# GJ0407790/cuda_ray_tracer

Measured on AMD Instinct MI355X. Metric: Mrays/sec, tenthousand.txt 1080p@16spp, higher is better.
Workload: dtype f32

## Files before the change

### cuda_ray_tracer_amd/csrc/api.hip

```cpp
#include "scene_dev.h"
#include "host_scene.h"

#include <cmath>
#include <cstdlib>
#include <cstring>
#include <new>
#include <string>
#include <vector>

using namespace mirt;

namespace {

template <typename T>
int upload(T** dst, const std::vector<T>& src)
{
  *dst = nullptr;
  if (src.empty()) return MIRT_OK;
  MIRT_HIP(hipMalloc(dst, sizeof(T) * src.size()));
  MIRT_HIP(hipMemcpy(*dst, src.data(), sizeof(T) * src.size(), hipMemcpyHostToDevice));
  return MIRT_OK;
}

bool nonzero(const MirtRGB& c) { return !(fabsf(c.r) < 1e-6f && fabsf(c.g) < 1e-6f && fabsf(c.b) < 1e-6f); }
// ... 151 lines not shown
  if (!std::isfinite(d->expose) && d->expose != INFINITY) sc->colors_finite = false;
  std::vector<LightDev> suns((size_t)d->num_suns), bulbs((size_t)d->num_bulbs);
  for (int i = 0; i < d->num_suns; ++i) {
    const MirtVec3& v = d->suns[i].dir;
    const float mag = sqrtf(v.x * v.x + v.y * v.y + v.z * v.z);
    float nx = 0.0f, ny = 0.0f, nz = 0.0f;
    const float diff = fabsf(mag - 0.0f), largest = fmaxf(fabsf(mag), fabsf(0.0f));
    const bool zero = (largest < 1e-6f) ? (diff < 1e-6f) : (diff / largest < 1e-6f);
    if (!zero) { const float inv = 1.0f / mag; nx = v.x * inv; ny = v.y * inv; nz = v.z * inv; }
    suns[i] = {v.x, v.y, v.z, d->suns[i].color.r, d->suns[i].color.g, d->suns[i].color.b, nx, ny, nz, 1.0f / nx, 1.0f / ny, 1.0f / nz};
  }
  for (int i = 0; i < d->num_bulbs; ++i) bulbs[i] = {d->bulbs[i].point.x, d->bulbs[i].point.y, d->bulbs[i].point.z, d->bulbs[i].color.r, d->bulbs[i].color.g, d->bulbs[i].color.b, 0, 0, 0, 0, 0, 0};
  sc->d.spheres = nullptr; sc->d.triangles = nullptr; sc->d.prim_refs = nullptr; sc->d.planes = nullptr; sc->d.suns = nullptr; sc->d.bulbs = nullptr;

  int rc = MIRT_OK;
  auto chk = [&](int r) { if (rc == MIRT_OK) rc = r; };
  {
    const size_t nodes_bytes = N > 1 ? 64 * (size_t)(N - 1) : 0;
    const size_t sph_bytes = 16 * (size_t)sc->Ns, tri_bytes = 48 * (size_t)sc->Nt;
    const size_t qnode_bytes = (sc->Nt == 0 && N > 1) ? 32 * (size_t)(N - 1) : 0;
    const size_t wnode_bytes = (sc->Nt > 0 && N > 1) ? 64 * (size_t)(N - 1) + 128 : 0;
    const size_t total = nodes_bytes + sph_bytes + tri_bytes + 64 + qnode_bytes + wnode_bytes;
    if (total > 0xfffffff0ull) { delete sc; set_error("mirt_scene_create: scene too large for 32-bit record offsets"); return MIRT_ERR_ARG; }
    hipError_t e = hipMalloc(&sc->heap, total);
    if (e == hipSuccess) e = hipMemset(sc->heap, 0, total);
    if (e != hipSuccess) { delete sc; return hip_fail(e, "hipMalloc(heap)", __FILE__, __LINE__); }
    sc->prim_base = (uint32_t)nodes_bytes;
    sc->qnode_base = qnode_bytes ? (uint32_t)(nodes_bytes + sph_bytes + tri_bytes + 64) : 0u;
    sc->wnode_base = wnode_bytes ? (uint32_t)((nodes_bytes + sph_bytes + tri_bytes + 64 + qnode_bytes + 127) / 128 * 128) : 0u;
    sc->nodes = reinterpret_cast<float4*>(sc->heap);
  }
  chk(upload(&sc->spheres, spheres)); chk(upload(&sc->tris, tris));
  chk(upload(&sc->tri_verts, verts)); chk(upload(&sc->mats, mats));
  chk(upload(&sc->refs_in, refs)); chk(upload(&sc->planes, planes)); chk(upload(&sc->suns, suns)); chk(upload(&sc->bulbs, bulbs));
  auto alloc = [&](void** p, size_t bytes) { if (rc == MIRT_OK && bytes) { hipError_t e = hipMalloc(p, bytes); if (e != hipSuccess) rc = hip_fail(e, "hipMalloc", __FILE__, __LINE__); } };
  if (N > 0) {
    alloc((void**)&sc->codes, 4 * (size_t)N); alloc((void**)&sc->order, 4 * (size_t)N);
    alloc((void**)&sc->parent, 4 * (2 * (size_t)N - 1)); alloc((void**)&sc->boxes, 24 * (2 * (size_t)N - 1));
    if (N > 1) { alloc((void**)&sc->child_l, 4 * (size_t)(N - 1)); alloc((void**)&sc->child_r, 4 * (size_t)(N - 1)); alloc((void**)&sc->range, 8 * (size_t)(N - 1)); }
    alloc((void**)&sc->unit_prim, 4 * ((size_t)sc->Ns + 3 * (size_t)sc->Nt));
    alloc((void**)&sc->tris_before, 4 * ((size_t)N + 1));
  }
  alloc((void**)&sc->bounds_keys, 6 * 4);
  alloc((void**)&sc->qparams, 9 * 4);
  alloc((void**)&sc->tri_boxes, 32 * (size_t)sc->Nt);
  for (int i = 0; i < mirt::MIRT_MAX_FRAMES; ++i) {
    alloc((void**)&sc->ctx[i].counters, 16 * sizeof(unsigned long long));
    if (rc == MIRT_OK && hipMemset(sc->ctx[i].counters, 0, 16 * sizeof(unsigned long long)) != hipSuccess) rc = MIRT_ERR_HIP;
  }
  if (rc == MIRT_OK) {
    hipError_t e = hipEventCreate(&sc->ev0);
    if (e == hipSuccess) e = hipEventCreate(&sc->ev1);
    if (e == hipSuccess) e = hipEventCreate(&sc->so_ev);
    for (int i = 0; i < mirt::MIRT_MAX_FRAMES && e == hipSuccess; ++i) {
      e = hipEventCreate(&sc->ctx[i].ev0);
      if (e == hipSuccess) e = hipEventCreate(&sc->ctx[i].ev1);
      if (e == hipSuccess) e = hipEventCreate(&sc->ctx[i].ev2);
      if (e == hipSuccess) e = hipEventCreate(&sc->ctx[i].ev3);
      if (e == hipSuccess) e = hipEventCreate(&sc->ctx[i].order_ev);
    }
    if (e != hipSuccess) rc = hip_fail(e, "hipEventCreate", __FILE__, __LINE__);
  }
  if (rc != MIRT_OK) { mirt_scene_destroy(sc); return rc; }
  *out = sc;
  return MIRT_OK;
}

}

extern "C" {

void mirt_scene_destroy(MirtScene* sc)
{
  if (!sc) return;
  hipSetDevice(sc->device);
  hipDeviceSynchronize();
  hipFree(sc->heap); hipFree(sc->spheres); hipFree(sc->tris); hipFree(sc->tri_verts); hipFree(sc->mats); hipFree(sc->refs_in);
  hipFree(sc->unit_prim); hipFree(sc->tris_before); hipFree(sc->range);
  hipFree(sc->planes); hipFree(sc->suns); hipFree(sc->bulbs);
  hipFree(sc->codes); hipFree(sc->order); hipFree(sc->child_l); hipFree(sc->child_r); hipFree(sc->parent); hipFree(sc->boxes); hipFree(sc->build_ws);
  hipFree(sc->bounds_keys); hipFree(sc->qparams); hipFree(sc->tri_boxes);
  for (int i = 0; i < mirt::MIRT_MAX_FRAMES; ++i) {
    mirt::RenderCtx& c = sc->ctx[i];
    hipFree(c.samples); hipFree(c.stack_spill); hipFree(c.pending); hipFree(c.counters); hipFree(c.args_dev);
    hipFree(c.chunk_cost); for (uint32_t* o : c.order_out) hipFree(o);
    hipFree(c.sp_list); hipFree(c.sp_table); hipFree(c.sp_blocks);
    if (c.ev0) hipEventDestroy(c.ev0);
    if (c.ev1) hipEventDestroy(c.ev1);
    if (c.ev2) hipEventDestroy(c.ev2);
    if (c.ev3) hipEventDestroy(c.ev3);
    if (c.order_ev) hipEventDestroy(c.order_ev);
    for (hipEvent_t e : c.slab_ev) hipEventDestroy(e);
  }
  rng_cache_free(&sc->rng);
  hipFree(sc->wf_state); hipFree(sc->wf_rays); hipFree(sc->wf_ctr);
  if (sc->wf_ctr_host) hipHostFree(sc->wf_ctr_host);
  for (hipEvent_t e : sc->wf_events) hipEventDestroy(e);
  if (sc->ev0) hipEventDestroy(sc->ev0);
  if (sc->ev1) hipEventDestroy(sc->ev1);
  if (sc->so_ev) hipEventDestroy(sc->so_ev);
  hipFree(sc->so_order); hipFree(sc->so_keys); hipFree(sc->so_keys2); hipFree(sc->so_ws);
  delete sc;
}

int mirt_build_lbvh(MirtScene* sc, void* stream, float* build_ms)
{
  if (!sc) { set_error("mirt_build_lbvh: null scene"); return MIRT_ERR_ARG; }
  MIRT_HIP(hipSetDevice(sc->device));
  int rc = build_lbvh(sc, (hipStream_t)stream);
  if (rc == MIRT_OK) sc->updated = false;
  if (rc == MIRT_OK && build_ms) *build_ms = sc->build_ms;
  return rc;
}

int64_t mirt_render_num_pixels(const MirtRenderParams* p) { return p ? render_num_pixels(p) : -1; }

int mirt_part_pixel_xy(const MirtRenderParams* p, int64_t local, int32_t* x, int32_t* y)
{
  if (!p) { set_error("mirt_part_pixel_xy: null argument"); return MIRT_ERR_ARG; }
  return part_pixel(p, local, x, y);
}

int mirt_render(MirtScene* sc, const MirtRenderParams* p, void* d_rgba8, void* d_rgba_f32, void* stream)
{
  if (!sc || !p) { set_error("mirt_render: null argument"); return MIRT_ERR_ARG; }
  MIRT_HIP(hipSetDevice(sc->device));
  return render(sc, p, d_rgba8, d_rgba_f32, (hipStream_t)stream);
}

int mirt_render_accumulate(MirtScene* sc, const MirtRenderParams* p, void* d_accum_f32, int sample_first, int sample_count, void* stream)
{
  if (!sc || !p) { set_error("mirt_render_accumulate: null argument"); return MIRT_ERR_ARG; }
  MIRT_HIP(hipSetDevice(sc->device));
  return render_accumulate(sc, p, d_accum_f32, sample_first, sample_count, (hipStream_t)stream);
}

int mirt_finalize(const MirtRenderParams* p, const void* d_accum_f32, int total_samples, void* d_rgba8, void* stream)
{
  if (!p) { set_error("mirt_finalize: null argument"); return MIRT_ERR_ARG; }
  return finalize(p, d_accum_f32, total_samples, d_rgba8, (hipStream_t)stream);
}

int mirt_render_accumulate_pixels(MirtScene* sc, const MirtRenderParams* p, const uint32_t* d_pixels, int64_t num_listed, void* d_accum_f32,
                                  void* d_accum_sq_f32, uint32_t* d_counts, int sample_first, int sample_count, void* stream)
{
  if (!sc || !p) { set_error("mirt_render_accumulate_pixels: null argument"); return MIRT_ERR_ARG; }
  if (!d_pixels && num_listed > 0) { set_error("mirt_render_accumulate_pixels: null pixel list (every pixel of the part: d_pixels = NULL with num_listed = 0)"); return MIRT_ERR_ARG; }
  MIRT_HIP(hipSetDevice(sc->device));
  mirt::AdaptiveArgs ax;
  ax.list = d_pixels; ax.num_listed = num_listed; ax.accum_sq = (float4*)d_accum_sq_f32; ax.counts = d_counts;
  return render_accumulate_pixels(sc, p, ax, d_accum_f32, sample_first, sample_count, (hipStream_t)stream);
}

int mirt_select_pixels(const MirtRenderParams* p, const void* d_accum_f32, const void* d_accum_sq_f32, const uint32_t* d_counts, int min_samples,
                       int max_samples, float max_variance, uint32_t* d_pixels_out, uint32_t* d_num_out, void* stream)
{
  if (!p) { set_error("mirt_select_pixels: null argument"); return MIRT_ERR_ARG; }
  return select_pixels(p, d_accum_f32, d_accum_sq_f32, d_counts, min_samples, max_samples, max_variance, d_pixels_out, d_num_out, (hipStream_t)stream);
}

int mirt_finalize_counts(const MirtRenderParams* p, const void* d_accum_f32, const uint32_t* d_counts, void* d_rgba8, void* stream)
{
  if (!p) { set_error("mirt_finalize_counts: null argument"); return MIRT_ERR_ARG; }
  return finalize_counts(p, d_accum_f32, d_counts, d_rgba8, (hipStream_t)stream);
}

int mirt_scatter_part(const MirtRenderParams* p, const void* d_part_rgba8, void* d_frame_rgba8, void* stream)
// ... 124 lines not shown
```

### cuda_ray_tracer_amd/csrc/render.hip

```cpp
#include "scene_dev.h"
#include "host_scene.h"
#include "shade_common.h"

#include <algorithm>
#include <climits>
#include <cmath>
#include <cstdio>
#include <cstdlib>
#include <cstring>

namespace mirt {
namespace {

constexpr int RBLOCK = 256;
constexpr int MAX_SPP = 4096;
constexpr int MAX_SLAB_ARGS = 4;
#ifndef MIRT_TRACE_BLOCK
#define MIRT_TRACE_BLOCK 64
#endif
constexpr int TRACE_BLOCK = MIRT_TRACE_BLOCK;
constexpr int MAX_CHUNK_SHIFT = 8, MIN_CHUNK_SHIFT = 6;
#ifndef MIRT_WAVES_PER_SIMD
#define MIRT_WAVES_PER_SIMD 4
#endif
#ifndef MIRT_STACK_LDS
#define MIRT_STACK_LDS 24
#endif
constexpr int STACK_LDS = MIRT_STACK_LDS;
MIRT_DEV bool triangle_leaf_reached(const RenderArgs* __restrict__ ap, uint32_t off16, const f3& o, const f3& d, float t, float tmin, f3& inv)
{
  const RenderArgs* aq = ap;
  asm volatile("" : "+s"(aq));
  const uint32_t id = aq->unit_prim[off16 - aq->prim_base16] & 0x7fffffffu;
  const float4 b0 = aq->tri_boxes[2 * (size_t)id], b1 = aq->tri_boxes[2 * (size_t)id + 1];
  inv = mk3(1.0f / d.x, 1.0f / d.y, 1.0f / d.z);
  const float tx1 = (b0.x - o.x) * inv.x, tx2 = (b0.y - o.x) * inv.x;
  const float ty1 = (b0.z - o.y) * inv.y, ty2 = (b0.w - o.y) * inv.y;
  const float tz1 = (b1.x - o.z) * inv.z, tz2 = (b1.y - o.z) * inv.z;
  const float te = fmaxf(fmaxf(fminf(tx1, tx2), fminf(ty1, ty2)), fminf(tz1, tz2));
  const float tx = fminf(fminf(fmaxf(tx1, tx2), fmaxf(ty1, ty2)), fmaxf(tz1, tz2));
  return te < tx && tx > tmin && te < t;
}

template <bool COUNT, int TABLES, bool QN, int SPECX = 0>
__global__ void __launch_bounds__(TRACE_BLOCK, MIRT_WAVES_PER_SIMD) trace_kernel(const RenderArgs* __restrict__ ap, const HotArgs h)
{
  constexpr int SPEC = SPECX;
  constexpr bool NOTRI = (SPEC & SPEC_NOTRI) != 0;
  constexpr bool WIDE = QN && !NOTRI;
#define MIRT_HELD (QN && !(SPEC & SPEC_NOBULB) && h.reach_check && S.batch_pending && !S.trav && S.li >= h.num_suns && S.li < h.num_suns + h.num_bulbs && \
                   S.refbest != REF_NONE)
  __shared__ __attribute__((aligned(16))) unsigned char lds_raw[STACK_LDS * TRACE_BLOCK * 4];
  __shared__ uint4 lds_rng[2][TRACE_BLOCK];
  __shared__ uint4 lds_park[2][TRACE_BLOCK];
  uint32_t* const lds_stack = reinterpret_cast<uint32_t*>(lds_raw);
  const int tid = threadIdx.x;
  const int lane = tid & 63;
  (void)lane;
  const unsigned char* const heap = reinterpret_cast<const unsigned char*>(h.nodes);
  const uint32_t gid32 = blockIdx.x * (uint32_t)TRACE_BLOCK + (uint32_t)tid;
  const long long gid = (long long)gid32;
  const long long gthreads = (long long)(gridDim.x * (uint32_t)TRACE_BLOCK);
  Counters cn = {0, 0, 0, 0, 0, 0, 0, 0, 0};

  unsigned long long c_next = 0, c_end = 0;
  bool exhausted = false;

  Lane S;
  S.g = -1; S.trav = false;
  S.rng.v0 = S.rng.v1 = S.rng.v2 = S.rng.v3 = S.rng.v4 = S.rng.d = 0; S.rng.bm_flag = 0; S.rng.bm_extra = 0.0f;
  S.L = mk3(0, 0, 0); S.alpha = 0.0f; S.steps = 0;
  S.Hdir = mk3(0, 0, 0); S.Hp = mk3(0, 0, 0); S.Hn = mk3(0, 0, 0); S.Hcolor = mk3(0, 0, 0);
  S.Hbounce = 0; S.Hior = 1.458f; S.Hrough = 0.0f; S.HtransNZ = false;
  S.wt = mk3(1, 1, 1); S.wD = mk3(0, 0, 0); S.pn = mk3(0, 0, 0);
  S.pc = 0; S.refr_bounce = 0; S.gi_n = 0; S.state = ST_PRIMARY;
  S.bo = mk3(0, 0, 0); S.rdir = mk3(0, 0, 1); S.li = 0; S.occl = 0ull; S.batch_pending = false; S.has_reflect = false;
  S.o = mk3(0, 0, 0); S.d = mk3(0, 0, 1); S.inv = mk3(0, 0, 1); S.bounce = 0; S.limit = INFINITY; S.shadow = false;
  S.tplane = INFINITY; S.plane_id = -1;
  S.qb = mk3(0, 0, 0); S.qc = mk3(0, 0, 0); S.qsx = S.qsy = S.qsz = 0;
  S.cur = REF_NONE; S.tos = REF_NONE; S.sp = 0; S.tbest = INFINITY; S.refbest = REF_NONE;

  lds_rng[0][tid] = make_uint4(0, 0, 0, 0);
  lds_rng[1][tid] = make_uint4(0, 0, 0, 0);
  lds_park[0][tid] = make_uint4(0, 0, 0, 0);
  lds_park[1][tid] = make_uint4(0, 0, 0, __float_as_uint(1.458f));
  for (;;) {
    const RenderArgs* aq = ap;
    asm volatile("" : "+s"(aq));
    const RenderArgs& a = *aq;
    if (a.reach_check && !S.trav && S.g >= 0 && !(exhausted && S.batch_pending && !MIRT_HELD) && (!S.batch_pending || S.li >= a.num_suns)) {
      if (hit_needs_literal_walk<QN>(a, S)) walk_literally<COUNT, NOTRI>(a, S, cn, gid, gthreads);
    }
    {
      const uint4 r0 = lds_rng[0][tid], r1 = lds_rng[1][tid];
      S.rng.v0 = r0.x; S.rng.v1 = r0.y; S.rng.v2 = r0.z; S.rng.v3 = r0.w;
      S.rng.v4 = r1.x; S.rng.d = r1.y; S.rng.bm_extra = __uint_as_float(r1.z); S.rng.bm_flag = (int)r1.w;
      const uint4 p0 = lds_park[0][tid], p1 = lds_park[1][tid];
      S.L = mk3(__uint_as_float(p0.x), __uint_as_float(p0.y), __uint_as_float(p0.z)); S.alpha = __uint_as_float(p0.w);
      S.wD = mk3(__uint_as_float(p1.x), __uint_as_float(p1.y), __uint_as_float(p1.z)); S.Hior = __uint_as_float(p1.w);
    }
    while (!S.trav && S.g >= 0 && !(exhausted && S.batch_pending && !MIRT_HELD)) {
      if (S.batch_pending) batch_next<COUNT, QN, RenderArgs, SPEC>(a, S, cn);
      else advance<COUNT, QN, SPEC>(a, S, cn, gid, gthreads);
    }
    if (!exhausted) {
      const unsigned long long need = __ballot(!S.trav && S.g < 0);
      if (need && (__popcll(need) >= a.init_k || __ballot(S.trav || S.batch_pending) == 0)) {
        const int want = __popcll(need);
        const unsigned long long nsamples = (unsigned long long)a.num_samples;
        const unsigned long long chunk = 1ull << a.chunk_shift;
        const unsigned long long nchunks = (nsamples + chunk - 1) >> a.chunk_shift;
        const int r = (int)__builtin_amdgcn_mbcnt_hi((unsigned)(need >> 32), __builtin_amdgcn_mbcnt_lo((unsigned)need, 0u));
        int given = 0;
        long long my = -1;
        while (given < want) {
          if (c_next >= c_end) {
            unsigned long long k = 0;
            if (lane == 0) {
              k = atomicAdd(a.work_counter, 1ull);
              if (k < nchunks && a.chunk_order) k = a.chunk_order[k];
            }
            k = __shfl(k, 0);
            if (k >= nchunks) {
              if (lane == 0 && atomicAdd(a.work_counter + 4, 1ull) == (unsigned long long)gridDim.x * (TRACE_BLOCK / 64) - 1ull) {
                a.work_counter[4] = 0ull;
                a.work_counter[0] = 0ull;
              }
              exhausted = true;
              break;
            }
            c_next = k << a.chunk_shift;
            c_end = (c_next + chunk < nsamples) ? c_next + chunk : nsamples;
          }
          const int avail = (int)(c_end - c_next);
          const int take = (want - given < avail) ? want - given : avail;
          if (!S.trav && S.g < 0 && r >= given && r < given + take) my = (long long)c_next + (r - given);
          c_next += (unsigned long long)take;
          given += take;
        }
        if (my >= 0) init_sample<COUNT, TABLES, QN>(a, S, cn, a.sample_order ? (long long)a.sample_order[my] : my);
      }
    }
    lds_rng[0][tid] = make_uint4(S.rng.v0, S.rng.v1, S.rng.v2, S.rng.v3);
    lds_rng[1][tid] = make_uint4(S.rng.v4, S.rng.d, __float_as_uint(S.rng.bm_extra), (uint32_t)S.rng.bm_flag);
    lds_park[0][tid] = make_uint4(__float_as_uint(S.L.x), __float_as_uint(S.L.y), __float_as_uint(S.L.z), __float_as_uint(S.alpha));
    lds_park[1][tid] = make_uint4(__float_as_uint(S.wD.x), __float_as_uint(S.wD.y), __float_as_uint(S.wD.z), __float_as_uint(S.Hior));
    if (__ballot(S.trav || S.batch_pending) == 0) {
      if (exhausted && __ballot(S.g >= 0) == 0) break;
      continue;
    }

    const float tmin = 0.0001f;
    for (;;) {
      const unsigned long long tm = __ballot(S.trav);
      const bool pend = !S.trav && S.batch_pending && !MIRT_HELD;
      const unsigned long long bm = __ballot(pend);
      if (tm == 0 && bm == 0) break;
      const int nwait = __popcll(__ballot(!S.trav && !pend && (S.g >= 0 || !exhausted)));
      const int nlive = __popcll(__ballot(S.g >= 0));
      const bool drain = exhausted && nlive <= h.drain_lanes;
      if (nwait >= h.refill_k || (drain && nwait > 0)) break;
      if (bm != 0 && (__popcll(bm) >= h.batch_k || tm == 0 || drain)) {
        if (pend) batch_next<COUNT, QN, HotArgs, SPEC>(h, S, cn);
      }
      const bool leaf0 = S.trav && (S.cur & REF_LEAF) != 0;
      const unsigned long long lm = __ballot(leaf0);
      const bool do_leaf0 = __popcll(lm) >= h.leaf_k || __ballot(S.trav && !leaf0) == 0 || drain;
      for (int rep = 0; rep < h.reps; ++rep) {
      const bool leaf = S.trav && (S.cur & REF_LEAF) != 0;
      const bool do_leaf = rep == 0 && do_leaf0;
      if (S.trav && (!leaf || do_leaf)) {
        if (COUNT) ++S.steps;
        const float4* rec = reinterpret_cast<const float4*>(heap + (S.cur << 4));
        bool pop = false;
        if (leaf) {
          float t = 0.0f;
          bool hit = false;
          const float4 q0 = rec[0];
          const bool tri = !NOTRI && (S.cur & REF_TRI) != 0;
          if (tri) {
            if (COUNT) cn.tri_tests++;
            const float4 q1 = rec[1], q2 = rec[2];
            hit = triangle_hit(q0, q1, q2, S.o, S.d, t);
          } else {
            if (COUNT) cn.sphere_tests++;
            float tc, t_far;
            hit = sphere_hit(q0, S.o, S.d, t, tc, t_far);
            if (QN && hit && (NOTRI || S.qsx != 0u)) hit = sphere_leaf_box_admits(q0, S.o, S.d, tc, t_far);
          }
          bool closer = closer_hit(hit, t, S.tbest, S.cur & REF_OFFMASK, S.refbest);
          if (QN && !NOTRI && closer && tri && S.qsx != 0u) {
            f3 inv;
            if (!triangle_leaf_reached(ap, S.cur & REF_OFFMASK, S.o, S.d, t, tmin, inv)) {
              closer = false;
              S.inv = inv; S.qsx = 0u;
              S.tos = 0u; S.sp = 1;
              S.tbest = INFINITY; S.refbest = REF_NONE;
            }
          }
          S.tbest = closer ? t : S.tbest;
          S.refbest = closer ? S.cur : S.refbest;
          S.trav = !(closer && S.shadow && t < S.limit);
          pop = S.trav;
        } else {
          if (COUNT) cn.internal_visits++;
          uint32_t noff = S.cur << 4;
          asm volatile("" : "+v"(noff));
          const float4* nrec = reinterpret_cast<const float4*>(heap + noff);
          bool hl, hr;
          float tel, ter;
          uint32_t lref, rref;
#define MIRT_PUSH(v) do { if (S.sp < h.lds_depth) lds_stack[S.sp * TRACE_BLOCK + tid] = S.tos; \
                          else h.stack_spill[(size_t)(S.sp - h.lds_depth) * gthreads + gid] = S.tos; \
                          S.tos = (v); ++S.sp; if (COUNT) cn.max_stack = max(cn.max_stack, (uint32_t)S.sp); } while (0)
          if (WIDE && S.qsx != 0u) {
            const uint4 w0 = *reinterpret_cast<const uint4*>(nrec), w1 = *reinterpret_cast<const uint4*>(nrec + 1);
            const uint4 w2 = *reinterpret_cast<const uint4*>(nrec + 2), w3 = *reinterpret_cast<const uint4*>(nrec + 3);
            const bool h0 = box_q(w0.x, w0.y, w0.z, S.inv, S.qb, S.qc, S.qsx, S.qsy, S.qsz, S.tbest, tmin);
            const bool h1 = box_q(w0.w, w1.x, w1.y, S.inv, S.qb, S.qc, S.qsx, S.qsy, S.qsz, S.tbest, tmin);
            const bool h2 = box_q(w1.z, w1.w, w2.x, S.inv, S.qb, S.qc, S.qsx, S.qsy, S.qsz, S.tbest, tmin);
            const bool h3 = box_q(w2.y, w2.z, w2.w, S.inv, S.qb, S.qc, S.qsx, S.qsy, S.qsz, S.tbest, tmin);
            uint32_t cand = w3.w;
            bool have = h3;
            if (h2 && have) MIRT_PUSH(cand);
            cand = h2 ? w3.z : cand; have = have || h2;
            if (h1 && have) MIRT_PUSH(cand);
            cand = h1 ? w3.y : cand; have = have || h1;
            hl = h0 || have; hr = h0 && have;
            lref = h0 ? w3.x : cand; rref = cand;
// ... 290 lines not shown
  }
  if ((int64_t)p->width * p->height > 0x7fffffffll - 1234) { set_error(std::string(who) + ": frame too large for the 32-bit pixel seed"); return MIRT_ERR_ARG; }
  if (npix == 0) return MIRT_OK;
  if (npix >= 0x7fffffffll || (long long)p->stripe_rows * p->width >= 0x7fffffffll) { set_error(std::string(who) + ": part too large"); return MIRT_ERR_ARG; }
  if (sparse && sc->opt.wavefront != 0) { set_error(std::string(who) + ": a pixel list is not supported with wavefront = 1 (the trace / shade kernel pair does not hand samples out through a table)"); return MIRT_ERR_ARG; }
  const bool per_pixel_seed = d_accum != nullptr || p->spp > 1;
  const int sppe = sample_count;
  const Options& opt = sc->opt;
  long long slab_pixels = (1ll << opt.slab_log2) / sppe;
  if (slab_pixels < 1) slab_pixels = 1;
  if (slab_pixels > npix) slab_pixels = npix;
  const int nslabs = (int)((npix + slab_pixels - 1) / slab_pixels);
  const long long slab_samples_max = slab_pixels * sppe;
  const long long listed_max = sparse ? (ax->num_listed < slab_pixels ? ax->num_listed : slab_pixels) : 0;
  const long long launch_samples_max = sparse ? listed_max * sppe : slab_samples_max;
  const bool count = (p->flags & MIRT_RENDER_COUNTERS) != 0;

  if (!sc->grid_blocks) sc->grid_blocks = grid_blocks(sc->device);
  const int blocks_cached = sc->grid_blocks;
  long long want_blocks = (launch_samples_max + TRACE_BLOCK - 1) / TRACE_BLOCK;
  int blocks = (int)(want_blocks < blocks_cached ? want_blocks : blocks_cached);
  if (!count && blocks == blocks_cached && launch_samples_max < 20ll * blocks_cached * TRACE_BLOCK) {
    for (int i = 0; i < MIRT_MAX_FRAMES; ++i) {
      const RenderCtx& c = sc->ctx[i];
      if (c.used && c.stream != stream && hipEventQuery(c.ev3) == hipErrorNotReady) { blocks = blocks_cached > 1 ? blocks_cached / 2 : 1; break; }
    }
  }
  if (opt.trace_waves >= 1 && opt.trace_waves <= blocks_cached) blocks = opt.trace_waves;
  const size_t gthreads = (size_t)blocks * TRACE_BLOCK;

  RenderCtx& cx = sc->ctx[sc->frame_no % MIRT_MAX_FRAMES];
  if (cx.used) {
    MIRT_HIP(hipEventSynchronize(cx.ev3));
    if (!cx.timed) {
      float ms = 0.0f;
      int rc = trace_ms_of(cx, &ms);
      if (rc != MIRT_OK) return rc;
      sc->trace_ms_sum += ms; sc->trace_frames += 1; cx.timed = true;
    }
  }
  if (cx.samples_cap < (size_t)slab_samples_max) {
    MIRT_HIP(hipStreamSynchronize(stream));
    hipFree(cx.samples); cx.samples = nullptr; cx.samples_cap = 0;
    MIRT_HIP(hipMalloc(&cx.samples, sizeof(float4) * (size_t)slab_samples_max));
    cx.samples_cap = (size_t)slab_samples_max;
  }
  const size_t spill_need = (size_t)STACK_TOTAL_WIDE * gthreads;
  if (cx.spill_cap < spill_need) {
    MIRT_HIP(hipStreamSynchronize(stream));
    hipFree(cx.stack_spill); cx.stack_spill = nullptr; cx.spill_cap = 0;
    MIRT_HIP(hipMalloc(&cx.stack_spill, sizeof(uint32_t) * spill_need));
    cx.spill_cap = spill_need;
  }
  if (sparse) {
    const size_t blocks_need = sparse_blocks_words(ax->num_listed);
    if (cx.sp_list_cap < (size_t)ax->num_listed || cx.sp_table_cap < (size_t)launch_samples_max || cx.sp_blocks_cap < blocks_need) {
      MIRT_HIP(hipStreamSynchronize(stream));
      if (cx.sp_list_cap < (size_t)ax->num_listed) {
        hipFree(cx.sp_list); cx.sp_list = nullptr; cx.sp_list_cap = 0;
        MIRT_HIP(hipMalloc(&cx.sp_list, 4 * (size_t)ax->num_listed));
        cx.sp_list_cap = (size_t)ax->num_listed;
      }
      if (cx.sp_table_cap < (size_t)launch_samples_max) {
        hipFree(cx.sp_table); cx.sp_table = nullptr; cx.sp_table_cap = 0;
        MIRT_HIP(hipMalloc(&cx.sp_table, 4 * (size_t)launch_samples_max));
        cx.sp_table_cap = (size_t)launch_samples_max;
      }
      if (cx.sp_blocks_cap < blocks_need) {
        hipFree(cx.sp_blocks); cx.sp_blocks = nullptr; cx.sp_blocks_cap = 0;
        MIRT_HIP(hipMalloc(&cx.sp_blocks, 4 * blocks_need));
        cx.sp_blocks_cap = blocks_need;
      }
    }
  }
  const bool need_pending = sc->any_trans || sc->d.gi != 0;
  const int pending_slots = need_pending ? 2 * (sc->d.bounces + (sc->d.gi > 0 ? sc->d.gi : 0) + 2) : 0;
  const size_t pending_need = (size_t)pending_slots * PENDING_WORDS * gthreads;
  if (cx.pending_cap < pending_need) {
    MIRT_HIP(hipStreamSynchronize(stream));
    hipFree(cx.pending); cx.pending = nullptr; cx.pending_cap = 0;
    MIRT_HIP(hipMalloc(&cx.pending, sizeof(float) * pending_need));
    cx.pending_cap = pending_need;
  }

  RenderArgs a;
  memset(&a, 0, sizeof(a));
  a.width = p->width; a.height = p->height; a.bounces = sc->d.bounces; a.gi = sc->d.gi;
  a.spp = d_accum ? (p->spp > 1 ? p->spp : 2) : p->spp;
  a.fisheye = sc->d.fisheye; a.panorama = sc->d.panorama;
  a.dof_focus = sc->d.dof_focus; a.dof_lens = sc->d.dof_lens; a.expose = sc->d.expose;
  a.forward.x = sc->d.forward.x; a.forward.y = sc->d.forward.y; a.forward.z = sc->d.forward.z;
  a.right.x = sc->d.right.x; a.right.y = sc->d.right.y; a.right.z = sc->d.right.z;
  a.up.x = sc->d.up.x; a.up.y = sc->d.up.y; a.up.z = sc->d.up.z;
  a.eye.x = sc->d.eye.x; a.eye.y = sc->d.eye.y; a.eye.z = sc->d.eye.z;
  a.stripe_rows = p->stripe_rows; a.num_parts = p->num_parts; a.part = p->part;
  a.sample_first = sample_first; a.sample_count = sample_count; a.seed_per_pixel = per_pixel_seed ? 1 : 0;
  a.nodes = sc->nodes; a.unit_prim = sc->unit_prim; a.mats = sc->mats;
  const bool notri = sc->Nt == 0;
  const bool qwant = opt.qnodes != 0 && opt.wavefront == 0;
  const bool qn = sc->grid_ok && (notri ? (qwant && opt.traversal >= 1 && sc->root_ref_q != REF_NONE)
                                        : (qwant && opt.traversal == 1 && sc->root_ref_w != REF_NONE && (opt.qnodes >= 2 || sc->N >= 65536)));
  const bool specialise = opt.specialise != 0 && sc->colors_finite;
  const bool nobulb = specialise && sc->d.num_bulbs == 0, nopend = specialise && !need_pending;
  a.root_ref = qn ? (notri ? sc->root_ref_q : sc->root_ref_w) : sc->root_ref; a.num_spheres = sc->Ns; a.num_prims = sc->N;
  a.qparams = qn ? sc->qparams : nullptr;
  a.tri_boxes = sc->tri_boxes;
  a.prim_base16 = sc->prim_base / 16u;
  a.swap_mask = opt.traversal == 1 ? ((qn && notri) ? NODE_SWAP_PURE : 0u) : (opt.traversal == 2 ? NODE_SWAP_ANY : 0u);
  a.skip_unlit = (opt.skip_unlit != 0 && sc->colors_finite && sc->d.num_suns + sc->d.num_bulbs <= 32) ? 1 : 0;
  a.shadow_anyhit = opt.shadow_anyhit != 0 ? 1 : 0;
  a.nonfinite_colours = sc->colors_finite ? 0 : 1;
  a.planes = sc->planes; a.num_planes = sc->d.num_planes;
  a.suns = sc->suns; a.num_suns = sc->d.num_suns;
  a.bulbs = sc->bulbs; a.num_bulbs = sc->d.num_bulbs;
  a.needs_rng = (a.spp >= 1) || (sc->d.dof_focus != 0.0f && !sc->d.fisheye && !sc->d.panorama) || sc->any_rough || sc->d.gi != 0;
  if (a.needs_rng) {
    int rc = ensure_rng_tables(&sc->rng, per_pixel_seed ? sample_first + sample_count : 0, (long long)p->width * p->height, stream, &a.rng, d_accum != nullptr);
    if (rc != MIRT_OK) return rc;
  }
  a.samples = cx.samples;
  a.stack_spill = cx.stack_spill;
  a.pending = cx.pending; a.pending_slots = pending_slots;
  a.counters = count ? cx.counters : nullptr;
  a.overflow = cx.counters + 9;
  a.lds_depth = (opt.stack_lds_depth >= 0 && opt.stack_lds_depth <= STACK_LDS) ? opt.stack_lds_depth : STACK_LDS;
  a.refill_k = opt.refill_k > 0 ? opt.refill_k : (qn ? (notri ? 32 : 24) : 64);
  a.drain_lanes = opt.drain_lanes;
  const int init_k = opt.init_k > 0 ? opt.init_k : (qn ? (notri ? 10 : 8) : 64);
  a.init_k = init_k < a.refill_k ? init_k : a.refill_k;
  a.batch_k = opt.batch_k;

  int chunk_shift = MAX_CHUNK_SHIFT;
  while (chunk_shift > MIN_CHUNK_SHIFT && (launch_samples_max >> chunk_shift) < 16ll * blocks * (TRACE_BLOCK / 64)) --chunk_shift;
  if (opt.chunk_shift >= 4) chunk_shift = opt.chunk_shift;
  a.chunk_shift = chunk_shift;
  const size_t nchunks = (size_t)((slab_samples_max + (1ll << chunk_shift) - 1) >> chunk_shift);
  const bool wavefront = opt.wavefront != 0;
  const bool sched = opt.sched == 1 && nslabs == 1 && !wavefront && !sparse;
  if (sched && cx.chunk_cap < nchunks) {
    MIRT_HIP(hipDeviceSynchronize());
    hipFree(cx.chunk_cost); cx.chunk_cost = nullptr; cx.chunk_cap = 0; cx.order_key = -1;
    for (uint32_t*& o : cx.order_out) { hipFree(o); o = nullptr; }
    MIRT_HIP(hipMalloc(&cx.chunk_cost, 4 * nchunks));
    for (uint32_t*& o : cx.order_out) MIRT_HIP(hipMalloc(&o, 4 * nchunks));
    cx.chunk_cap = nchunks;
  }
  const long long okey = slab_samples_max * 16 + chunk_shift;
  const uint32_t* order = nullptr;
  if (sched) {
    unsigned long long best = 0;
    for (int i = 0; i < MIRT_MAX_FRAMES; ++i) {
      RenderCtx& c = sc->ctx[i];
      if (&c == &cx || !c.used || c.order_key != okey || c.order_frame <= best) continue;
      if (hipEventQuery(c.order_ev) != hipSuccess) continue;
      best = c.order_frame; order = c.order_out[(c.order_writes - 1) % RenderCtx::ORDER_BUFS];
    }
    if (!order && cx.used && cx.order_key == okey) order = cx.order_out[(cx.order_writes - 1) % RenderCtx::ORDER_BUFS];
  }
  const long long total_samples = (long long)npix * sppe;
  const bool by_sample = opt.sched == 2 && !wavefront && !sparse && slab_samples_max < 0x7fffffffll && total_samples <= (3ll << 30);
  bool measure_samples = false, ordered_samples = false;
  a.sample_order = nullptr; a.sample_key = nullptr;
  if (by_sample) {
    order = nullptr;
    if (sc->so_busy && hipEventQuery(sc->so_ev) == hipSuccess) sc->so_busy = false;
    if (sc->so_key == okey && sc->so_total == total_samples && !sc->so_busy) ordered_samples = true;
    else if (!sc->so_busy) {
      for (int i = 0; i < MIRT_MAX_FRAMES; ++i) if (sc->ctx[i].used) MIRT_HIP(hipEventSynchronize(sc->ctx[i].ev3));
      if (sc->so_cap < (size_t)total_samples || sc->so_slab_cap < (size_t)slab_samples_max) {
        hipFree(sc->so_order); hipFree(sc->so_keys); hipFree(sc->so_keys2); hipFree(sc->so_ws);
        sc->so_order = sc->so_keys = sc->so_keys2 = sc->so_ws = nullptr; sc->so_cap = 0; sc->so_slab_cap = 0; sc->so_key = -1;
        const bool got = hipMalloc(&sc->so_order, 4 * (size_t)total_samples) == hipSuccess && hipMalloc(&sc->so_keys, 4 * (size_t)slab_samples_max) == hipSuccess &&
                         hipMalloc(&sc->so_keys2, 4 * (size_t)slab_samples_max) == hipSuccess && hipMalloc(&sc->so_ws, 4 * sort_low_byte_ws_words(slab_samples_max)) == hipSuccess;
        if (got) { sc->so_cap = (size_t)total_samples; sc->so_slab_cap = (size_t)slab_samples_max; }
        else {
          (void)hipGetLastError();
          hipFree(sc->so_order); hipFree(sc->so_keys); hipFree(sc->so_keys2); hipFree(sc->so_ws);
          sc->so_order = sc->so_keys = sc->so_keys2 = sc->so_ws = nullptr;
        }
      }
      if (sc->so_cap >= (size_t)total_samples && sc->so_slab_cap >= (size_t)slab_samples_max) {
        measure_samples = true;
        sc->so_key = -1;
        sc->so_pending_key = okey; sc->so_total = total_samples;
      }
    }
  }
  const bool measure = (sched && !by_sample && !order) || measure_samples;
  a.chunk_order = order;
  a.chunk_cost = (measure && !by_sample) ? cx.chunk_cost : nullptr;
  cx.frame_id = ++sc->frame_seq;
  MIRT_HIP(hipEventRecord(cx.ev0, stream));
  if (measure && !by_sample) MIRT_HIP(hipMemsetAsync(cx.chunk_cost, 0, 4 * nchunks, stream));
  if (count) { MIRT_HIP(hipMemsetAsync(cx.counters, 0, 8 * sizeof(unsigned long long), stream)); MIRT_HIP(hipMemsetAsync(cx.counters + 11, 0, sizeof(unsigned long long), stream)); }
  a.work_counter = cx.counters + 8;
  cx.wf_trace_ms = -1.0f;
  float wf_ms_total = 0.0f;
  HotArgs h;
  h.nodes = a.nodes; h.root_ref = a.root_ref; h.swap_mask = a.swap_mask; h.qparams = a.qparams;
  h.planes = a.planes; h.num_planes = a.num_planes; h.suns = a.suns; h.num_suns = a.num_suns; h.bulbs = a.bulbs; h.num_bulbs = a.num_bulbs; h.shadow_anyhit = a.shadow_anyhit;
  h.stack_spill = a.stack_spill; h.lds_depth = a.lds_depth; h.refill_k = a.refill_k; h.batch_k = a.batch_k; h.drain_lanes = a.drain_lanes;
  a.reach_check = (qn && sc->N > 1) ? 1 : 0;
  a.reach_slack = 4.76837158203125e-07f * sc->coord_max;
  h.reach_check = a.reach_check;
  h.leaf_k = opt.leaf_k > 0 ? opt.leaf_k : (qn ? 8 : 4);
// ... 205 lines not shown
```

### cuda_ray_tracer_amd/csrc/scene_dev.h

```cpp
#ifndef MIRT_SCENE_DEV_H
#define MIRT_SCENE_DEV_H

#include <hip/hip_runtime.h>
#include <string>
#include <vector>

#include "../../include/mirt.h"
#include "device_common.h"
#include "xorwow_tables.h"

namespace mirt {

constexpr uint32_t REF_LEAF = 0x80000000u;
constexpr uint32_t REF_TRI = 0x40000000u;
constexpr uint32_t REF_OFFMASK = 0x0fffffffu;
constexpr uint32_t REF_NONE = 0xf0000000u;
constexpr float QGRID = 65535.0f;
constexpr uint32_t REF_QPURE = 0x20000000u;
constexpr uint32_t QBOX_NONE = 0x0000ffffu;
constexpr int STACK_TOTAL_WIDE = 88;
constexpr float QINV_STEPS = 1152921504606846976.0f;
constexpr uint32_t NODE_SWAP_PURE = 1u;
constexpr uint32_t NODE_SWAP_ANY = 2u;

struct PlaneDev { float nx, ny, nz, px, py, pz; float mat[11]; float pad; };
struct LightDev { float x, y, z, r, g, b; float nx, ny, nz, ix, iy, iz; };

struct RenderArgs {
  int width, height, bounces, spp, gi;
  int fisheye, panorama;
  float dof_focus, dof_lens, expose;
  f3 forward, right, up, eye;
  int stripe_rows, num_parts, part;
  long long num_local_pixels;
  long long num_samples;
  long long pixel_base;
  int sample_first;
  int sample_count;
  int seed_per_pixel;
  const float4* nodes;
  const uint32_t* unit_prim;
  const float4* mats;
  uint32_t root_ref;
  uint32_t prim_base16;
  uint32_t swap_mask;
  int reach_check;
  float reach_slack;
  int skip_unlit;
  int shadow_anyhit;
  const float* qparams;
  const float4* tri_boxes;
  int num_spheres;
  int num_prims;
  const PlaneDev* planes; int num_planes;
  int nonfinite_colours;
  const LightDev* suns; int num_suns;
  const LightDev* bulbs; int num_bulbs;
  RngTablesDev rng;
  int needs_rng;
  float4* samples;
  uint32_t* stack_spill;
  float* pending;
  int pending_slots;
  int refill_k;
  int lds_depth;
  int drain_lanes;
  int batch_k;
  int init_k;
  unsigned long long* counters;
  unsigned long long* overflow;
  unsigned long long* work_counter;
  const uint32_t* chunk_order;
  int chunk_shift;
  uint32_t* chunk_cost;
  const uint32_t* sample_order;
  uint32_t* sample_key;
};

struct HotArgs {
  const float4* nodes;
  uint32_t root_ref;
  uint32_t swap_mask;
  const float* qparams;
  const PlaneDev* planes; int num_planes;
  const LightDev* suns; int num_suns;
  const LightDev* bulbs; int num_bulbs;
  int shadow_anyhit;
  uint32_t* stack_spill;
  int lds_depth, refill_k, batch_k, drain_lanes;
  int reps;
  int leaf_k;
  int reach_check;
};

struct ResolveArgs {
  const float4* samples;
  unsigned char* rgba8;
  float4* rgba_f32;
  float4* accum;
  long long num_local_pixels;
  long long pixel_base;
  int spp;
  int count;
};

struct RngCache {
  RngTables host;
  long long key = -1;
  uint4* A = nullptr; uint32_t* B = nullptr; uint32_t* K = nullptr; uint32_t* R2 = nullptr;
};

struct Options {
  int bounds_as_shipped = 0;
  int traversal = 1;
  int wavefront = 0;
  int stack_lds_depth = -1;
  int refill_k = 0;
  int batch_k = 8, drain_lanes = 16;
  int leaf_k = 0;
  int reps = 0;
  int init_k = 0;
  int chunk_shift = 0;
  int trace_waves = 0;
  int shadow_anyhit = 1;
  int skip_unlit = 1;
  int qnodes = 1;
  int specialise = 1;
  int sched = 2;
  int slab_log2 = 28;
  int wf_pool = 1 << 21, wf_refill_k = 16;
};

constexpr int MIRT_MAX_FRAMES = 4;
struct RenderCtx {
  float4* samples = nullptr; size_t samples_cap = 0;
  uint32_t* stack_spill = nullptr; size_t spill_cap = 0;
  float* pending = nullptr; size_t pending_cap = 0;
  unsigned long long* counters = nullptr;
  hipStream_t stream = nullptr;
  RenderArgs* args_dev = nullptr;
  RenderArgs args_host[4];
  bool args_valid[4] = {false, false, false, false};
  hipEvent_t ev0 = nullptr, ev1 = nullptr, ev2 = nullptr, ev3 = nullptr;
  std::vector<hipEvent_t> slab_ev;
  int launches = 0;
  int node_bytes = 64;
  bool used = false, counted = false, timed = true;
  uint32_t* chunk_cost = nullptr;
  static constexpr unsigned ORDER_BUFS = 3;
  uint32_t* order_out[ORDER_BUFS] = {nullptr, nullptr, nullptr};
  size_t chunk_cap = 0;
  unsigned uses = 0;
  unsigned long long frame_id = 0;
  long long order_key = -1;
  unsigned order_writes = 0;
  unsigned long long order_frame = 0;
  hipEvent_t order_ev = nullptr;
  float wf_trace_ms = -1.0f;
  uint32_t* sp_list = nullptr; size_t sp_list_cap = 0;
  uint32_t* sp_table = nullptr; size_t sp_table_cap = 0;
  uint32_t* sp_blocks = nullptr; size_t sp_blocks_cap = 0;
};

struct AdaptiveArgs {
  const uint32_t* list = nullptr;
  long long num_listed = 0;
  float4* accum_sq = nullptr;
  uint32_t* counts = nullptr;
};

}

struct MirtScene {
  int device = 0;
  MirtSceneDesc d{};
  int N = 0, Ns = 0, Nt = 0;
  mirt::Options opt;
  int grid_blocks = 0, wf_trace_blocks = 0;
  float4* spheres = nullptr;
  float4* tris = nullptr;
  float4* mats = nullptr;
  MirtPrimRef* refs_in = nullptr;
  float4* tri_verts = nullptr;
  mirt::PlaneDev* planes = nullptr;
  mirt::LightDev* suns = nullptr;
  mirt::LightDev* bulbs = nullptr;
  uint32_t* codes = nullptr;
  uint32_t* order = nullptr;
  uint32_t* child_l = nullptr;
  uint32_t* child_r = nullptr;
  int* parent = nullptr;
  float* boxes = nullptr;
  float4* nodes = nullptr;
  unsigned char* heap = nullptr;
  uint32_t prim_base = 0;
  uint32_t* unit_prim = nullptr;
  uint32_t* tris_before = nullptr;
  uint2* range = nullptr;
  uint32_t qnode_base = 0;
  uint32_t wnode_base = 0;
  uint32_t root_ref_w = mirt::REF_NONE;
  uint32_t root_ref_q = mirt::REF_NONE;
  float* qparams = nullptr;
  float4* tri_boxes = nullptr;
  uint32_t* build_ws = nullptr; size_t build_ws_words = 0;
  uint32_t* bounds_keys = nullptr;
  uint32_t root_ref = mirt::REF_NONE;
  bool built = false;
  float build_ms = 0.0f;
  float coord_max = 0.0f;
  bool grid_ok = false;
  mirt::RenderCtx ctx[mirt::MIRT_MAX_FRAMES];
  unsigned frame_no = 0;
  unsigned long long frame_seq = 0;
  mirt::RenderCtx* last = nullptr;
  unsigned long long overflow_events = 0;
  double trace_ms_sum = 0.0; int trace_frames = 0;
  uint32_t* wf_state = nullptr; size_t wf_state_cap = 0;
  float4* wf_rays = nullptr; size_t wf_rays_cap = 0;
  unsigned long long* wf_ctr = nullptr;
// ... 49 lines not shown
```

Before: 8254.

## Stage precomputed primary rays in a per-wave global pool for refill

When a wave refills idle lanes, it now fills a full 64-record per-wave ring buffer in global memory, using all lanes to initialize samples and compute primary-ray setup (rng state, origin, direction, inverse, plane, quantized box). Idle lanes then pop ready records instead of each running init_sample only for the lanes that need work. The aim is to replace refills that run with few active lanes by full-wave batched initialization. In exchange it adds global-memory traffic for the stage pool and extra bookkeeping packed into pool_state. The LDS park and rng writes also move to before the refill.

```diff
diff --git a/cuda_ray_tracer_amd/csrc/api.hip b/cuda_ray_tracer_amd/csrc/api.hip
--- a/cuda_ray_tracer_amd/csrc/api.hip
+++ b/cuda_ray_tracer_amd/csrc/api.hip
@@ -257,7 +257,7 @@
   hipFree(sc->bounds_keys); hipFree(sc->qparams); hipFree(sc->tri_boxes);
   for (int i = 0; i < mirt::MIRT_MAX_FRAMES; ++i) {
     mirt::RenderCtx& c = sc->ctx[i];
-    hipFree(c.samples); hipFree(c.stack_spill); hipFree(c.pending); hipFree(c.counters); hipFree(c.args_dev);
+    hipFree(c.samples); hipFree(c.stack_spill); hipFree(c.pending); hipFree(c.stage_pool); hipFree(c.counters); hipFree(c.args_dev);
     hipFree(c.chunk_cost); for (uint32_t* o : c.order_out) hipFree(o);
     hipFree(c.sp_list); hipFree(c.sp_table); hipFree(c.sp_blocks);
     if (c.ev0) hipEventDestroy(c.ev0);
diff --git a/cuda_ray_tracer_amd/csrc/render.hip b/cuda_ray_tracer_amd/csrc/render.hip
--- a/cuda_ray_tracer_amd/csrc/render.hip
+++ b/cuda_ray_tracer_amd/csrc/render.hip
@@ -65,6 +65,7 @@
 
   unsigned long long c_next = 0, c_end = 0;
   bool exhausted = false;
+  uint32_t pool_state = 0;
 
   Lane S;
   S.g = -1; S.trav = false;
@@ -103,48 +104,111 @@
       if (S.batch_pending) batch_next<COUNT, QN, RenderArgs, SPEC>(a, S, cn);
       else advance<COUNT, QN, SPEC>(a, S, cn, gid, gthreads);
     }
+    lds_rng[0][tid] = make_uint4(S.rng.v0, S.rng.v1, S.rng.v2, S.rng.v3);
+    lds_rng[1][tid] = make_uint4(S.rng.v4, S.rng.d, __float_as_uint(S.rng.bm_extra), (uint32_t)S.rng.bm_flag);
+    lds_park[0][tid] = make_uint4(__float_as_uint(S.L.x), __float_as_uint(S.L.y), __float_as_uint(S.L.z), __float_as_uint(S.alpha));
+    lds_park[1][tid] = make_uint4(__float_as_uint(S.wD.x), __float_as_uint(S.wD.y), __float_as_uint(S.wD.z), __float_as_uint(S.Hior));
     if (!exhausted) {
       const unsigned long long need = __ballot(!S.trav && S.g < 0);
       if (need && (__popcll(need) >= a.init_k || __ballot(S.trav || S.batch_pending) == 0)) {
         const int want = __popcll(need);
-        const unsigned long long nsamples = (unsigned long long)a.num_samples;
-        const unsigned long long chunk = 1ull << a.chunk_shift;
-        const unsigned long long nchunks = (nsamples + chunk - 1) >> a.chunk_shift;
+        int pool_head = (int)(pool_state & 0xffu), pool_count = (int)((pool_state >> 8) & 0xffu);
+        bool queue_done = (pool_state >> 16) != 0u;
+        uint4* const pw = a.stage_pool + (size_t)(blockIdx.x * (uint32_t)(TRACE_BLOCK / 64) + (uint32_t)__builtin_amdgcn_readfirstlane(tid >> 6)) * (STAGE_QUARTERS * STAGE_RECORDS);
+        if (pool_count < want && !queue_done) {
+          const int room = STAGE_RECORDS - pool_count;
+          const unsigned long long nsamples = (unsigned long long)a.num_samples;
+          const unsigned long long chunk = 1ull << a.chunk_shift;
+          const unsigned long long nchunks = (nsamples + chunk - 1) >> a.chunk_shift;
+          int given = 0;
+          int my = -1;
+          while (given < room) {
+            if (c_next >= c_end) {
+              unsigned long long k = 0;
+              if (lane == 0) {
+                k = atomicAdd(a.work_counter, 1ull);
+                if (k < nchunks && a.chunk_order) k = a.chunk_order[k];
+              }
+              k = __shfl(k, 0);
+              if (k >= nchunks) {
+                if (lane == 0 && atomicAdd(a.work_counter + 4, 1ull) == (unsigned long long)gridDim.x * (TRACE_BLOCK / 64) - 1ull) {
+                  a.work_counter[4] = 0ull;
+                  a.work_counter[0] = 0ull;
+                }
+                queue_done = true;
+                break;
+              }
+              c_next = k << a.chunk_shift;
+              c_end = (c_next + chunk < nsamples) ? c_next + chunk : nsamples;
+            }
+            const int avail = (int)(c_end - c_next);
+            const int take = (room - given < avail) ? room - given : avail;
+            if (lane >= given && lane < given + take) my = (int)c_next + (lane - given);
+            c_next += (unsigned long long)take;
+            given += take;
+          }
+          if (my >= 0) {
+            const long long idx = (long long)(a.sample_order ? a.sample_order[my] : (uint32_t)my);
+            Lane T;
+            init_sample_core<COUNT, TABLES>(a, T, cn, idx);
+            if (a.bounces == 0) {
+              a.samples[idx] = make_float4(0.0f, 0.0f, 0.0f, 0.0f);
+              if (COUNT && a.sample_key) a.sample_key[idx] = 255u;
+            } else {
+              uint4* const rec = pw + ((pool_head + pool_count + lane) & (STAGE_RECORDS - 1));
+              rec[0 * STAGE_RECORDS] = make_uint4((uint32_t)T.g, T.rng.v0, T.rng.v1, T.rng.v2);
+              rec[1 * STAGE_RECORDS] = make_uint4(T.rng.v3, T.rng.v4, T.rng.d, __float_as_uint(T.rng.bm_extra));
+              rec[2 * STAGE_RECORDS] = make_uint4((uint32_t)T.rng.bm_flag, __float_as_uint(T.o.x), __float_as_uint(T.o.y), __float_as_uint(T.o.z));
+              asm volatile("" ::: "memory");
+              start_ray<COUNT, false, QN>(a, T, cn);
+              rec[3 * STAGE_RECORDS] = make_uint4(__float_as_uint(T.d.x), __float_as_uint(T.d.y), __float_as_uint(T.d.z), __float_as_uint(T.tplane));
+              rec[4 * STAGE_RECORDS] = make_uint4(__float_as_uint(T.inv.x), __float_as_uint(T.inv.y), __float_as_uint(T.inv.z),
+                                                  ((uint32_t)(T.plane_id + 1) << 1) | (T.trav ? 1u : 0u));
+              if (QN) {
+                rec[5 * STAGE_RECORDS] = make_uint4(__float_as_uint(T.qb.x), __float_as_uint(T.qb.y), __float_as_uint(T.qb.z), __float_as_uint(T.qc.x));
+                rec[6 * STAGE_RECORDS] = make_uint4(__float_as_uint(T.qc.y), __float_as_uint(T.qc.z), 0u, 0u);
+              }
+            }
+          }
+          if (a.bounces != 0) pool_count += given;
+          __builtin_amdgcn_fence(__ATOMIC_RELEASE, "workgroup");
+          __builtin_amdgcn_fence(__ATOMIC_ACQUIRE, "workgroup");
+        }
+        const int n = want < pool_count ? want : pool_count;
         const int r = (int)__builtin_amdgcn_mbcnt_hi((unsigned)(need >> 32), __builtin_amdgcn_mbcnt_lo((unsigned)need, 0u));
-        int given = 0;
-        long long my = -1;
-        while (given < want) {
-          if (c_next >= c_end) {
-            unsigned long long k = 0;
-            if (lane == 0) {
-              k = atomicAdd(a.work_counter, 1ull);
-              if (k < nchunks && a.chunk_order) k = a.chunk_order[k];
-            }
-            k = __shfl(k, 0);
-            if (k >= nchunks) {
-              if (lane == 0 && atomicAdd(a.work_counter + 4, 1ull) == (unsigned long long)gridDim.x * (TRACE_BLOCK / 64) - 1ull) {
-                a.work_counter[4] = 0ull;
-                a.work_counter[0] = 0ull;
-              }
-              exhausted = true;
-              break;
-            }
-            c_next = k << a.chunk_shift;
-            c_end = (c_next + chunk < nsamples) ? c_next + chunk : nsamples;
+        if (!S.trav && S.g < 0 && r < n) {
+          const uint4* const rec = pw + ((pool_head + r) & (STAGE_RECORDS - 1));
+          const uint4 q0 = rec[0 * STAGE_RECORDS], q1 = rec[1 * STAGE_RECORDS], q2 = rec[2 * STAGE_RECORDS], q3 = rec[3 * STAGE_RECORDS], q4 = rec[4 * STAGE_RECORDS];
+          S.g = (int)q0.x;
+          S.steps = 0;
+          S.pc = 0; S.state = ST_PRIMARY; S.limit = INFINITY; S.shadow = false; S.batch_pending = false;
+          lds_rng[0][tid] = make_uint4(q0.y, q0.z, q0.w, q1.x);
+          lds_rng[1][tid] = make_uint4(q1.y, q1.z, q1.w, q2.x);
+          lds_park[0][tid] = make_uint4(0u, 0u, 0u, 0u);
+          S.o = mk3(__uint_as_float(q2.y), __uint_as_float(q2.z), __uint_as_float(q2.w));
+          S.d = mk3(__uint_as_float(q3.x), __uint_as_float(q3.y), __uint_as_float(q3.z));
+          S.bounce = a.bounces;
+          S.tplane = __uint_as_float(q3.w);
+          S.inv = mk3(__uint_as_float(q4.x), __uint_as_float(q4.y), __uint_as_float(q4.z));
+          S.plane_id = (int)(q4.w >> 1) - 1;
+          S.trav = (q4.w & 1u) != 0u;
+          if (QN) {
+            const uint4 q5 = rec[5 * STAGE_RECORDS], q6 = rec[6 * STAGE_RECORDS];
+            S.qb = mk3(__uint_as_float(q5.x), __uint_as_float(q5.y), __uint_as_float(q5.z));
+            S.qc = mk3(__uint_as_float(q5.w), __uint_as_float(q6.x), __uint_as_float(q6.y));
+            S.qsx = S.inv.x >= 0.0f ? 0x07060100u : 0x07060302u;
+            S.qsy = S.inv.y >= 0.0f ? 0x07060100u : 0x07060302u;
+            S.qsz = S.inv.z >= 0.0f ? 0x07060100u : 0x07060302u;
           }
-          const int avail = (int)(c_end - c_next);
-          const int take = (want - given < avail) ? want - given : avail;
-          if (!S.trav && S.g < 0 && r >= given && r < given + take) my = (long long)c_next + (r - given);
-          c_next += (unsigned long long)take;
-          given += take;
+          S.tbest = INFINITY; S.refbest = REF_NONE;
+          S.cur = a.root_ref; S.sp = 0;
         }
-        if (my >= 0) init_sample<COUNT, TABLES, QN>(a, S, cn, a.sample_order ? (long long)a.sample_order[my] : my);
-      }
-    }
-    lds_rng[0][tid] = make_uint4(S.rng.v0, S.rng.v1, S.rng.v2, S.rng.v3);
-    lds_rng[1][tid] = make_uint4(S.rng.v4, S.rng.d, __float_as_uint(S.rng.bm_extra), (uint32_t)S.rng.bm_flag);
-    lds_park[0][tid] = make_uint4(__float_as_uint(S.L.x), __float_as_uint(S.L.y), __float_as_uint(S.L.z), __float_as_uint(S.alpha));
-    lds_park[1][tid] = make_uint4(__float_as_uint(S.wD.x), __float_as_uint(S.wD.y), __float_as_uint(S.wD.z), __float_as_uint(S.Hior));
+        pool_head = (pool_head + n) & (STAGE_RECORDS - 1);
+        pool_count -= n;
+        exhausted = queue_done && pool_count == 0;
+        pool_state = (uint32_t)pool_head | ((uint32_t)pool_count << 8) | (queue_done ? 0x10000u : 0u);
+      }
+    }
     if (__ballot(S.trav || S.batch_pending) == 0) {
       if (exhausted && __ballot(S.g >= 0) == 0) break;
       continue;
@@ -601,6 +665,13 @@
     MIRT_HIP(hipMalloc(&cx.pending, sizeof(float) * pending_need));
     cx.pending_cap = pending_need;
   }
+  const size_t stage_need = opt.wavefront != 0 ? 0 : (gthreads / 64) * (size_t)(STAGE_QUARTERS * STAGE_RECORDS);
+  if (cx.stage_cap < stage_need) {
+    MIRT_HIP(hipStreamSynchronize(stream));
+    hipFree(cx.stage_pool); cx.stage_pool = nullptr; cx.stage_cap = 0;
+    MIRT_HIP(hipMalloc(&cx.stage_pool, sizeof(uint4) * stage_need));
+    cx.stage_cap = stage_need;
+  }
 
   RenderArgs a;
   memset(&a, 0, sizeof(a));
@@ -640,6 +711,7 @@
   a.samples = cx.samples;
   a.stack_spill = cx.stack_spill;
   a.pending = cx.pending; a.pending_slots = pending_slots;
+  a.stage_pool = cx.stage_pool;
   a.counters = count ? cx.counters : nullptr;
   a.overflow = cx.counters + 9;
   a.lds_depth = (opt.stack_lds_depth >= 0 && opt.stack_lds_depth <= STACK_LDS) ? opt.stack_lds_depth : STACK_LDS;
diff --git a/cuda_ray_tracer_amd/csrc/scene_dev.h b/cuda_ray_tracer_amd/csrc/scene_dev.h
--- a/cuda_ray_tracer_amd/csrc/scene_dev.h
+++ b/cuda_ray_tracer_amd/csrc/scene_dev.h
@@ -18,6 +18,8 @@
 constexpr float QGRID = 65535.0f;
 constexpr uint32_t REF_QPURE = 0x20000000u;
 constexpr uint32_t QBOX_NONE = 0x0000ffffu;
+constexpr int STAGE_RECORDS = 64;
+constexpr int STAGE_QUARTERS = 7;
 constexpr int STACK_TOTAL_WIDE = 88;
 constexpr float QINV_STEPS = 1152921504606846976.0f;
 constexpr uint32_t NODE_SWAP_PURE = 1u;
@@ -62,6 +64,7 @@
   uint32_t* stack_spill;
   float* pending;
   int pending_slots;
+  uint4* stage_pool;
   int refill_k;
   int lds_depth;
   int drain_lanes;
@@ -136,6 +139,7 @@
   float4* samples = nullptr; size_t samples_cap = 0;
   uint32_t* stack_spill = nullptr; size_t spill_cap = 0;
   float* pending = nullptr; size_t pending_cap = 0;
+  uint4* stage_pool = nullptr; size_t stage_cap = 0;
   unsigned long long* counters = nullptr;
   hipStream_t stream = nullptr;
   RenderArgs* args_dev = nullptr;
```

Measured after the change: 8164. 0.989x the previous value.
